# atx/padne

Measured on AMD Instinct MI355X. Metric: CG solves/s, higher is better.
Workload: dtype f64; 1 GPU; C4 8-layer N=10M: 8-layer jittered triangular Laplacian, 9999392 nodes, via-ring stitched, 1 A source/sink, amg-PCG to rtol 1e-12; n_unknowns=9999391, nnz_per_rank=69955225, rows_per_rank=9999391, parallelism=layer-partitioned x1

## Files before the change

padne_amd/csrc/pcg.hip:

```cpp
#include "common.hpp"

#include <algorithm>
#include <math.h>
#include <stdlib.h>
#include <string.h>
#include <vector>

namespace padne {

__device__ __forceinline__ double wave_sum_v(double v) {
#pragma unroll
    for (int off = 32; off > 0; off >>= 1) v += __shfl_down(v, off, 64);
    return v;
}

__device__ __forceinline__ double block_total(const double *__restrict__ partials, int P, double *red) {
    double s = 0.0;
    for (int i = threadIdx.x; i < P; i += 256) s += partials[i];
    s = wave_sum_v(s);
    const int lane = threadIdx.x & 63, w = threadIdx.x >> 6;
    if (lane == 0) red[w] = s;
    __syncthreads();
    const double t = (red[0] + red[1]) + (red[2] + red[3]);
    __syncthreads();
    return t;
}

__device__ __forceinline__ void block_total2(const double *__restrict__ pa, const int Pa, const double *__restrict__ pb, const int Pb,
                                             double *red2, double *ta, double *tb) {
    double sa = 0.0, sb = 0.0;
    const int P = Pa > Pb ? Pa : Pb;
    for (int i = threadIdx.x; i < P; i += 256) {
        if (i < Pa) sa += pa[i];
        if (i < Pb) sb += pb[i];
    }
    sa = wave_sum_v(sa);
    sb = wave_sum_v(sb);
    const int lane = threadIdx.x & 63, w = threadIdx.x >> 6;
    if (lane == 0) {
        red2[w] = sa;
        red2[4 + w] = sb;
    }
    __syncthreads();
    *ta = (red2[0] + red2[1]) + (red2[2] + red2[3]);
    *tb = (red2[4] + red2[5]) + (red2[6] + red2[7]);
    __syncthreads();
}

__device__ __forceinline__ void block_store_partial(double v, double *red, double *out) {
    v = wave_sum_v(v);
    const int lane = threadIdx.x & 63, w = threadIdx.x >> 6;
    if (lane == 0) red[w] = v;
    __syncthreads();
    if (threadIdx.x == 0) *out = (red[0] + red[1]) + (red[2] + red[3]);
    __syncthreads();
}

struct PcgStatus {
    int32_t done;
    int32_t code;
    int32_t iters;
    int32_t done_seen;
    double rr;
    double tol2;
    double bb;
};

__global__ __launch_bounds__(256) void pcg_init_kernel(
    const long long n, const double *__restrict__ b, const double *__restrict__ ax,
    const double *__restrict__ dinv, double *__restrict__ r, double *__restrict__ p,
    double *__restrict__ part_rz, double *__restrict__ part_rr, double *__restrict__ part_bb) {
    __shared__ double red[4];
    double rz = 0.0, rr = 0.0, bb = 0.0;
    for (long long i = (long long)blockIdx.x * 256 + threadIdx.x; i < n; i += (long long)gridDim.x * 256) {
        const double bi = b[i];
        const double ri = ax ? bi - ax[i] : bi;
        const double zi = dinv[i] * ri;
        r[i] = ri;
        p[i] = zi;
        rz += ri * zi;
        rr += ri * ri;
        bb += bi * bi;
    }
    block_store_partial(rz, red, part_rz + blockIdx.x);
    block_store_partial(rr, red, part_rr + blockIdx.x);
    block_store_partial(bb, red, part_bb + blockIdx.x);
}

__global__ __launch_bounds__(256) void fold_partials_kernel(const double *__restrict__ partials, int P,
                                                            int stride, int count, double *__restrict__ out) {
    __shared__ double red[4];
    for (int c = 0; c < count; ++c) {
        const double t = block_total(partials + (size_t)c * stride, P, red);
        if (threadIdx.x == 0) out[c] = t;
    }
}

__global__ void pcg_set_tolerance_kernel(PcgStatus *st, const double *__restrict__ scal_rr_bb, double rtol,
                                         double atol, int use_existing_bb) {
    const double bb = use_existing_bb ? st->bb : scal_rr_bb[1];
    const double rr = scal_rr_bb[0];
    double tol = rtol * sqrt(bb);
    if (atol > tol) tol = atol;
    st->bb = bb;
    st->tol2 = tol * tol;
    st->rr = rr;
    st->code = PADNE_OK;
    st->done = (rr <= tol * tol) ? 1 : 0;
    if (!(rr == rr)) {
        st->done = 1;
        st->code = PADNE_E_BREAKDOWN;
    }
}

__global__ __launch_bounds__(256) void pcg_update_xr_kernel(
    const long long n, const double *__restrict__ part_rz, const int P_rz,
    const double *__restrict__ part_pq, const int P_pq, const double *__restrict__ p,
    const double *__restrict__ q, const double *__restrict__ dinv, double *__restrict__ x,
    double *__restrict__ r, double *__restrict__ part_rz_new, double *__restrict__ part_rr,
    PcgStatus *__restrict__ st) {
    __shared__ double red[4];
    if (st->done) return;
    const double rz = block_total(part_rz, P_rz, red);
    const double pq = block_total(part_pq, P_pq, red);
    const double alpha = rz / pq;
    double s_rz = 0.0, s_rr = 0.0;
    for (long long i = (long long)blockIdx.x * 256 + threadIdx.x; i < n; i += (long long)gridDim.x * 256) {
        const double pi = p[i];
        const double ri = r[i] - alpha * q[i];
        if (x != nullptr) x[i] += alpha * pi;
        r[i] = ri;
        const double zi = dinv[i] * ri;
        s_rz += ri * zi;
        s_rr += ri * ri;
    }
    block_store_partial(s_rz, red, part_rz_new + blockIdx.x);
    block_store_partial(s_rr, red, part_rr + blockIdx.x);
}

__global__ __launch_bounds__(256) void pcg_update_p_kernel(
    const long long n, const double *__restrict__ part_rz_new, const double *__restrict__ part_rz_old,
    const int P_rz, const double *__restrict__ part_rr, const int P_rr,
    const double *__restrict__ part_pq, const int P_pq, const double *__restrict__ r,
    const double *__restrict__ dinv, double *__restrict__ p, PcgStatus *__restrict__ st,
    const int max_iter, double *__restrict__ rec_next = nullptr, double *__restrict__ rec_pq = nullptr) {
    __shared__ double red[4];
    if (st->done) return;
    const double rz_new = block_total(part_rz_new, P_rz, red);
    const double rz_old = block_total(part_rz_old, P_rz, red);
    const double beta = rz_new / rz_old;
    for (long long i = (long long)blockIdx.x * 256 + threadIdx.x; i < n; i += (long long)gridDim.x * 256) {
        p[i] = dinv[i] * r[i] + beta * p[i];
    }
    if (blockIdx.x == 0) {
        const double rr = block_total(part_rr, P_rr, red);
        const double pq = block_total(part_pq, P_pq, red);
        if (threadIdx.x == 0 && rec_next != nullptr) {
            rec_next[0] = rz_new;
            rec_next[1] = rr;
            rec_pq[0] = pq;
        }
        __syncthreads();
        if (threadIdx.x == 0) {
            const int it = st->iters + 1;
            st->iters = it;
            st->rr = rr;
            if (!(pq > 0.0) || !(rr == rr)) {
                st->code = PADNE_E_BREAKDOWN;
                st->done = 1;
            } else if (rr <= st->tol2 || it >= max_iter) {
                st->done = 1;
            }
        }
    }
}

__global__ __launch_bounds__(256) void residual_kernel(const long long n, const double *__restrict__ b,
                                                       const double *__restrict__ ax, double *__restrict__ r,
                                                       double *__restrict__ part_rr) {
    __shared__ double red[4];
    double rr = 0.0;
    for (long long i = (long long)blockIdx.x * 256 + threadIdx.x; i < n; i += (long long)gridDim.x * 256) {
        const double ri = ax[i] - b[i];
        if (r) r[i] = -ri;
        rr += ri * ri;
    }
    block_store_partial(rr, red, part_rr + blockIdx.x);
}

__global__ __launch_bounds__(256) void pcg_update_xr_plain_kernel(
    const long long n, const double *__restrict__ part_rz, const int P_rz, const double *__restrict__ part_pq,
    const int P_pq, const double *__restrict__ p, const double *__restrict__ q, double *__restrict__ x,
    double *__restrict__ r, double *__restrict__ part_rr, PcgStatus *__restrict__ st) {
    __shared__ double red[4];
    const int stop = st->done;
    if (blockIdx.x == 0 && threadIdx.x == 0) st->done_seen = stop;
    if (stop) return;
    const double rz = block_total(part_rz, P_rz, red);
    const double pq = block_total(part_pq, P_pq, red);
    const double alpha = rz / pq;
    double s_rr = 0.0;
    for (long long i = (long long)blockIdx.x * 256 + threadIdx.x; i < n; i += (long long)gridDim.x * 256) {
        const double ri = r[i] - alpha * q[i];
        x[i] += alpha * p[i];
        r[i] = ri;
        s_rr += ri * ri;
    }
    block_store_partial(s_rr, red, part_rr + blockIdx.x);
}

__global__ __launch_bounds__(256) void pcg_update_xr_entry_kernel(
    const long long n, const double *__restrict__ part_rz, const int P_rz, const double *__restrict__ part_pq,
    const int P_pq, const double *__restrict__ p, const double *__restrict__ q, double *__restrict__ x,
    double *__restrict__ r, double *__restrict__ part_rr, PcgStatus *__restrict__ st, const double *__restrict__ bb2,
    const float c, const float *__restrict__ dinv32, float *__restrict__ b32, float *__restrict__ xa32, const int p_hat) {
    __shared__ double red[8];
    const int stop = st->done;
    if (blockIdx.x == 0 && threadIdx.x == 0) st->done_seen = stop;
    if (stop) return;
    double rz, pq;
    block_total2(part_rz, P_rz, part_pq, P_pq, red, &rz, &pq);
    const double s2 = *bb2;
    const double s_inv = s2 > 0.0 ? 1.0 / sqrt(s2) : 1.0;
    const double alpha = p_hat ? rz / (pq * (s2 > 0.0 ? sqrt(s2) : 1.0)) : rz / pq;
    double s_rr = 0.0;
    for (long long i = (long long)blockIdx.x * 256 + threadIdx.x; i < n; i += (long long)gridDim.x * 256) {
        const double ri = r[i] - alpha * q[i];
        if (x != nullptr) x[i] += alpha * p[i];
        r[i] = ri;
        s_rr += ri * ri;
        const float v = (float)(ri * s_inv);
        b32[i] = v;
        if (xa32 != nullptr) xa32[i] = c * dinv32[i] * v;
    }
    block_store_partial(s_rr, red, part_rr + blockIdx.x);
}

__global__ void p_hat_from_z_kernel(const long long n, const double *__restrict__ z, const double *__restrict__ bb2, float *__restrict__ p32) {
    const double s2 = *bb2;
    const double s_inv = s2 > 0.0 ? 1.0 / sqrt(s2) : 1.0;
    for (long long i = (long long)blockIdx.x * blockDim.x + threadIdx.x; i < n; i += (long long)gridDim.x * blockDim.x)
        p32[i] = (float)(z[i] * s_inv);
}

__global__ __launch_bounds__(256) void pcg_update_p_z_kernel(
    const long long n, const double *__restrict__ part_rz_new, const double *__restrict__ part_rz_old,
    const int P_rz, const double *__restrict__ part_rr, const int P_rr, const double *__restrict__ part_pq,
    const int P_pq, const double *__restrict__ z, double *__restrict__ p, PcgStatus *__restrict__ st,
    const int max_iter, double *__restrict__ x_deferred, const float *__restrict__ z32, const double *__restrict__ bb2,
    float *__restrict__ p32, float *__restrict__ p32_next = nullptr, double *__restrict__ alpha_out = nullptr) {
    __shared__ double red[8];
    if (st->done_seen) return;
    double rz_new, rz_old;
    block_total2(part_rz_new, P_rz, part_rz_old, P_rz, red, &rz_new, &rz_old);
    const double beta = rz_new / rz_old;
    if (z32 != nullptr) {
        const double s2 = *bb2;
        const double z_mul = s2 > 0.0 ? sqrt(s2) : 1.0;
        const bool need_alpha = p32_next == nullptr || blockIdx.x == 0;
        const double alpha = need_alpha ? rz_old / block_total(part_pq, P_pq, red) : 0.0;
        if (p32 != nullptr) {
            const double alpha_hat = alpha / z_mul;
            if (p32_next != nullptr) {
                if (blockIdx.x == 0 && threadIdx.x == 0) *alpha_out = alpha_hat;
                for (long long i = (long long)blockIdx.x * 256 + threadIdx.x; i < n; i += (long long)gridDim.x * 256)
                    p32_next[i] = (float)((double)z32[i] + beta * (double)p32[i]);
            } else {
                for (long long i = (long long)blockIdx.x * 256 + threadIdx.x; i < n; i += (long long)gridDim.x * 256) {
                    const double pi = (double)p32[i];
                    x_deferred[i] += alpha_hat * pi;
                    p32[i] = (float)((double)z32[i] + beta * pi);
                }
            }
        } else {
            for (long long i = (long long)blockIdx.x * 256 + threadIdx.x; i < n; i += (long long)gridDim.x * 256) {
                const double pi = p[i];
                x_deferred[i] += alpha * pi;
                p[i] = (double)z32[i] * z_mul + beta * pi;
            }
        }
    } else if (x_deferred != nullptr) {
        const double alpha = rz_old / block_total(part_pq, P_pq, red);
        for (long long i = (long long)blockIdx.x * 256 + threadIdx.x; i < n; i += (long long)gridDim.x * 256) {
            const double pi = p[i];
            x_deferred[i] += alpha * pi;
            p[i] = z[i] + beta * pi;
        }
    } else {
        for (long long i = (long long)blockIdx.x * 256 + threadIdx.x; i < n; i += (long long)gridDim.x * 256)
            p[i] = z[i] + beta * p[i];
    }
    if (blockIdx.x == 0) {
        const double rr = block_total(part_rr, P_rr, red);
        const double pq = block_total(part_pq, P_pq, red);
        __syncthreads();
        if (threadIdx.x == 0) {
            const int it = st->iters + 1;
            st->iters = it;
            st->rr = rr;
            if (!(pq > 0.0) || !(rr == rr) || !(rz_new > 0.0)) {
                st->code = PADNE_E_BREAKDOWN;
                st->done = 1;
            } else if (rr <= st->tol2 || it >= max_iter) {
                st->done = 1;
            }
        }
    }
}

__global__ __launch_bounds__(256) void pcg_x_flush_kernel(const long long n, const float *__restrict__ hist, const size_t slot_stride,
                                                          const int n_slots, const double *__restrict__ alpha, const int j0,
                                                          const int j1, const PcgStatus *__restrict__ st, double *__restrict__ x) {
    __shared__ double a_s[64];
    __shared__ int s_s[64];
    const int hi = min(j1, st->iters);
    const int cnt = hi - j0;
    if (cnt <= 0) return;
    if ((int)threadIdx.x < cnt && threadIdx.x < 64) {
        a_s[threadIdx.x] = alpha[(j0 + threadIdx.x) % n_slots];
        s_s[threadIdx.x] = (j0 + threadIdx.x) % n_slots;
    }
    __syncthreads();
    for (long long i = (long long)blockIdx.x * 256 + threadIdx.x; i < n; i += (long long)gridDim.x * 256) {
        double xi = x[i];
        int k = 0;
        for (; k + 4 <= cnt; k += 4) {
            const float p0 = hist[(size_t)s_s[k] * slot_stride + i], p1 = hist[(size_t)s_s[k + 1] * slot_stride + i],
                        p2 = hist[(size_t)s_s[k + 2] * slot_stride + i], p3 = hist[(size_t)s_s[k + 3] * slot_stride + i];
            xi += a_s[k] * (double)p0;
            xi += a_s[k + 1] * (double)p1;
            xi += a_s[k + 2] * (double)p2;
            xi += a_s[k + 3] * (double)p3;
        }
        for (; k < cnt; ++k) xi += a_s[k] * (double)hist[(size_t)s_s[k] * slot_stride + i];
        x[i] = xi;
    }
}

__global__ __launch_bounds__(256) void pcg_init_plain_kernel(const long long n, const double *__restrict__ b,
                                                             const double *__restrict__ ax, double *__restrict__ r,
                                                             double *__restrict__ part_rr,
                                                             double *__restrict__ part_bb) {
    __shared__ double red[4];
    double rr = 0.0, bb = 0.0;
    for (long long i = (long long)blockIdx.x * 256 + threadIdx.x; i < n; i += (long long)gridDim.x * 256) {
        const double bi = b[i];
        const double ri = ax ? bi - ax[i] : bi;
        r[i] = ri;
        rr += ri * ri;
        bb += bi * bi;
    }
    block_store_partial(rr, red, part_rr + blockIdx.x);
    block_store_partial(bb, red, part_bb + blockIdx.x);
}

static int vec_grid(long long n) {
    long long g = (n + 255) / 256;
    if (g > 1024) g = 1024;
    if (g < 1) g = 1;
    return (int)g;
}

enum { SLOT_PQ = 0, SLOT_RZ0 = 1, SLOT_RZ1 = 2, SLOT_RR = 3, SLOT_BB = 4, SLOT_TMP = 5 };
static inline double *slot(padne_ctx *ctx, int s) { return ctx->partials + (size_t)s * kMaxPartials; }

template <typename T>
__global__ void halo_pack_kernel(T *__restrict__ v, const int *__restrict__ export_idx, int n_export,
                                 long long dst_offset, const int *__restrict__ done_flag) {
    if (done_flag != nullptr && *done_flag != 0) return;
    const int k = blockIdx.x * blockDim.x + threadIdx.x;
    if (k < n_export) v[dst_offset + k] = v[export_idx[k]];
}

enum { S_RR = 0, S_BB = 1, S_TRUE = 2,
       S_NRM = 3,
       S_PQ = 8, S_RZRR0 = 10, S_RZRR1 = 12 };

template <typename T>
__global__ void halo_store_peers_kernel(const T *__restrict__ v, const int *__restrict__ export_idx, int n_export, void *const *peers,
                                        size_t entry_off, int world, int rank, int m_cap, const int *__restrict__ done_flag,
                                        unsigned long long seq1) {
    if (done_flag != nullptr && *done_flag != 0) return;
    const int k = blockIdx.x * blockDim.x + threadIdx.x;
    if (k < n_export) {
        const T val = v[export_idx[k]];
        for (int q = 0; q < world; ++q) {
            T *cell = reinterpret_cast<T *>(static_cast<char *>(peers[q]) + entry_off + ((size_t)rank * m_cap + k) * 8);
            if (seq1 != 0ull)
                __hip_atomic_store(cell, val, __ATOMIC_RELAXED, __HIP_MEMORY_SCOPE_SYSTEM);
            else
                *cell = val;
        }
    }
    if (seq1 == 0ull) return;
    __threadfence_system();
    __syncthreads();
    __shared__ int s_last;
    if (threadIdx.x == 0) {
        unsigned int *counter = reinterpret_cast<unsigned int *>(static_cast<char *>(peers[rank]) + kP2pCounterOff);
        const unsigned int prev = __hip_atomic_fetch_add(counter, 1u, __ATOMIC_ACQ_REL, __HIP_MEMORY_SCOPE_AGENT);
        s_last = prev + 1u == gridDim.x ? 1 : 0;
        if (s_last) __hip_atomic_store(counter, 0u, __ATOMIC_RELAXED, __HIP_MEMORY_SCOPE_AGENT);
    }
    __syncthreads();
    if (s_last && (int)threadIdx.x < world) {
        unsigned long long *flag = reinterpret_cast<unsigned long long *>(static_cast<char *>(peers[threadIdx.x])) + rank;
        __hip_atomic_store(flag, seq1, __ATOMIC_RELEASE, __HIP_MEMORY_SCOPE_SYSTEM);
    }
}

template <typename T>
__global__ void halo_unpack_kernel(T *__restrict__ v, long long n_owned, int m, int world, const void *mbox, size_t entry_off,
                                   int m_cap, const int *__restrict__ done_flag, unsigned long long seq1,
                                   unsigned long long timeout_ticks) {
    if (done_flag != nullptr && *done_flag != 0) return;
    if (seq1 != 0ull) {
        if ((int)threadIdx.x < world) {
            const unsigned long long *flag = static_cast<const unsigned long long *>(mbox) + threadIdx.x;
            const unsigned long long t0 = wall_clock64();
            while (__hip_atomic_load(flag, __ATOMIC_ACQUIRE, __HIP_MEMORY_SCOPE_SYSTEM) < seq1) {
                if (wall_clock64() - t0 > timeout_ticks) {
                    unsigned long long *err = reinterpret_cast<unsigned long long *>(const_cast<char *>(static_cast<const char *>(mbox)) + kP2pErrorOff);
                    __hip_atomic_store(err, ((unsigned long long)(threadIdx.x + 1) << 48) | (seq1 & 0xffffffffffffull), __ATOMIC_RELAXED,
                                       __HIP_MEMORY_SCOPE_SYSTEM);
                    break;
                }
                __builtin_amdgcn_s_sleep(32);
            }
        }
        __syncthreads();
    }
    const int j = blockIdx.x * blockDim.x + threadIdx.x;
    if (j >= world * m) return;
    const int r = j / m, k = j - r * m;
    const T *cell = reinterpret_cast<const T *>(static_cast<const char *>(mbox) + entry_off + ((size_t)r * m_cap + k) * 8);
    v[n_owned + j] = seq1 != 0ull ? __hip_atomic_load(cell, __ATOMIC_RELAXED, __HIP_MEMORY_SCOPE_SYSTEM) : *cell;
}

template <typename T>
static int halo_send_t(padne_ctx *ctx, const HaloPlan &plan, T *v, const int32_t *done_flag, HaloTicket *tk) {
    tk->p2p = false;
    if (plan.m <= 0) return PADNE_OK;
    if (comm_p2p_enabled(ctx) && comm_p2p_fits(ctx, plan.m)) {
        void **peers = nullptr;
        PADNE_TRY(comm_p2p_begin(ctx, plan.m, &peers, &tk->entry_off));
        tk->p2p = true;
        tk->seq1 = ctx->p2p_ipc ? ctx->p2p_seq : 0ull;
        if (plan.n_export > 0 || ctx->p2p_ipc) {
            hipLaunchKernelGGL(halo_store_peers_kernel<T>, dim3(plan.n_export > 0 ? (plan.n_export + 255) / 256 : 1), dim3(256), 0,
                               ctx->stream, (const T *)v, plan.export_idx, plan.n_export, (void *const *)peers, tk->entry_off,
                               ctx->world, ctx->rank, ctx->p2p_m_cap, done_flag, tk->seq1);
            PADNE_HIP_CHECK(hipGetLastError());
        }
        return PADNE_OK;
    }
    const long long seg_off = plan.n_owned + (long long)ctx->rank * plan.m;
    if (plan.n_export > 0) {
        hipLaunchKernelGGL(halo_pack_kernel<T>, dim3((plan.n_export + 255) / 256), dim3(256), 0, ctx->stream, v,
                           plan.export_idx, plan.n_export, seg_off, done_flag);
        PADNE_HIP_CHECK(hipGetLastError());
    }
    return PADNE_OK;
}

static int allgather_t(padne_ctx *ctx, const double *send, double *recv, int count) { return comm_allgather_f64(ctx, send, recv, count); }
static int allgather_t(padne_ctx *ctx, const float *send, float *recv, int count) { return comm_allgather_f32(ctx, send, recv, count); }

template <typename T>
static int halo_recv_t(padne_ctx *ctx, const HaloPlan &plan, T *v, const int32_t *done_flag, const HaloTicket &tk) {
    if (plan.m <= 0) return PADNE_OK;
    if (tk.p2p) {
        PADNE_TRY(comm_p2p_arrive(ctx));
        const int n = ctx->world * plan.m;
        hipLaunchKernelGGL(halo_unpack_kernel<T>, dim3((n + 255) / 256), dim3(256), 0, ctx->stream, v, plan.n_owned, plan.m,
                           ctx->world, (const void *)ctx->p2p_mbox, tk.entry_off, ctx->p2p_m_cap, done_flag, tk.seq1,
                           (unsigned long long)ctx->p2p_timeout_ms * 100000ull);
        PADNE_HIP_CHECK(hipGetLastError());
        return PADNE_OK;
    }
    const long long seg_off = plan.n_owned + (long long)ctx->rank * plan.m;
    return allgather_t(ctx, v + seg_off, v + plan.n_owned, plan.m);
}

int halo_send(padne_ctx *ctx, const HaloPlan &plan, double *v, const int32_t *done_flag, HaloTicket *tk) { return halo_send_t(ctx, plan, v, done_flag, tk); }
int halo_send_f32(padne_ctx *ctx, const HaloPlan &plan, float *v, const int32_t *done_flag, HaloTicket *tk) { return halo_send_t(ctx, plan, v, done_flag, tk); }
int halo_recv(padne_ctx *ctx, const HaloPlan &plan, double *v, const int32_t *done_flag, const HaloTicket &tk) { return halo_recv_t(ctx, plan, v, done_flag, tk); }
int halo_recv_f32(padne_ctx *ctx, const HaloPlan &plan, float *v, const int32_t *done_flag, const HaloTicket &tk) { return halo_recv_t(ctx, plan, v, done_flag, tk); }

int halo_exchange_plan(padne_ctx *ctx, const HaloPlan &plan, double *v, const int32_t *done_flag) {
    HaloTicket tk;
    PADNE_TRY(halo_send(ctx, plan, v, done_flag, &tk));
    return halo_recv(ctx, plan, v, done_flag, tk);
}

int halo_exchange_plan_f32(padne_ctx *ctx, const HaloPlan &plan, float *v, const int32_t *done_flag) {
    HaloTicket tk;
    PADNE_TRY(halo_send_f32(ctx, plan, v, done_flag, &tk));
    return halo_recv_f32(ctx, plan, v, done_flag, tk);
}

static int halo_exchange(padne_ctx *ctx, double *v, const int32_t *done_flag) {
    if (!ctx->halo_on) return PADNE_OK;
    HaloPlan plan;
    plan.n_owned = ctx->halo_n_owned;
    plan.m = ctx->halo_m;
    plan.n_export = ctx->halo_n_export;
    plan.export_idx = ctx->halo_export;
    return halo_exchange_plan(ctx, plan, v, done_flag);
}

}
extern "C" int padne_ctx_halo_exchange_time(padne_ctx *ctx, int32_t repeats, double *seconds_out) {
    using namespace padne;
    PADNE_REQUIRE(ctx && seconds_out && repeats > 0, "argument");
    PADNE_REQUIRE(ctx->halo_on, "no halo plan on this context");
    PADNE_HIP_CHECK(hipSetDevice(ctx->device));
    const size_t n = (size_t)ctx->halo_n_owned + (size_t)ctx->world * (size_t)ctx->halo_m;
    double *v = (double *)pool_alloc(ctx, sizeof(double) * (n ? n : 1));
    if (v == nullptr) return PADNE_E_NOMEM;
    int rc = PADNE_OK;
    hipError_t e = hipMemsetAsync(v, 0, sizeof(double) * n, ctx->stream);
    for (int k = 0; k < 3 && rc == PADNE_OK && e == hipSuccess; ++k) rc = halo_exchange(ctx, v, nullptr);
    if (e == hipSuccess) e = hipEventRecord(ctx->ev0, ctx->stream);
    for (int k = 0; k < repeats && rc == PADNE_OK && e == hipSuccess; ++k) rc = halo_exchange(ctx, v, nullptr);
    if (e == hipSuccess) e = hipEventRecord(ctx->ev1, ctx->stream);
    if (e == hipSuccess) e = hipEventSynchronize(ctx->ev1);
    float ms = 0.f;
    if (e == hipSuccess) e = hipEventElapsedTime(&ms, ctx->ev0, ctx->ev1);
    pool_free(ctx, v);
    if (e != hipSuccess) {
        set_error("halo exchange timing failed: %s", hipGetErrorString(e));
        return PADNE_E_HIP;
    }
    PADNE_TRY(rc);
    PADNE_TRY(comm_p2p_check(ctx));
    *seconds_out = (double)ms * 1e-3 / repeats;
    return PADNE_OK;
}
extern "C" int padne_test_halo_exchange(padne_ctx *ctx, int32_t as_float, const double *x_host, double *out_host) {
    using namespace padne;
    PADNE_REQUIRE(ctx && x_host && out_host, "null argument");
    PADNE_REQUIRE(ctx->halo_on, "no halo plan on this context");
    PADNE_HIP_CHECK(hipSetDevice(ctx->device));
    const size_t n_owned = (size_t)ctx->halo_n_owned, n = n_owned + (size_t)ctx->world * (size_t)ctx->halo_m;
    const size_t elem = as_float ? sizeof(float) : sizeof(double);
    HaloPlan plan;
    plan.n_owned = ctx->halo_n_owned;
    plan.m = ctx->halo_m;
    plan.n_export = ctx->halo_n_export;
    plan.export_idx = ctx->halo_export;
    std::vector<float> h32(as_float ? n : 0);
    for (size_t i = 0; as_float && i < n_owned; ++i) h32[i] = (float)x_host[i];
    void *v = pool_alloc(ctx, elem * (n ? n : 1));
    if (v == nullptr) return PADNE_E_NOMEM;
    int rc = PADNE_OK;
    hipError_t e = hipMemsetAsync(v, 0xff, elem * n, ctx->stream);
    if (e == hipSuccess && n_owned > 0)
        e = hipMemcpyAsync(v, as_float ? (const void *)h32.data() : (const void *)x_host, elem * n_owned, hipMemcpyHostToDevice,
                           ctx->stream);
    if (e == hipSuccess) rc = as_float ? halo_exchange_plan_f32(ctx, plan, (float *)v, nullptr) : halo_exchange_plan(ctx, plan, (double *)v, nullptr);
    if (e == hipSuccess && rc == PADNE_OK && n > 0)
        e = hipMemcpyAsync(as_float ? (void *)h32.data() : (void *)out_host, v, elem * n, hipMemcpyDeviceToHost, ctx->stream);
    const hipError_t es = hipStreamSynchronize(ctx->stream);
    if (e == hipSuccess) e = es;
    pool_free(ctx, v);
    if (e != hipSuccess) {
        set_error("halo exchange failed: %s", hipGetErrorString(e));
        return PADNE_E_HIP;
    }
    PADNE_TRY(rc);
    PADNE_TRY(comm_p2p_check(ctx));
    for (size_t i = 0; as_float && i < n; ++i) out_host[i] = (double)h32[i];
    return PADNE_OK;
}
namespace padne {

static int halo_product_dot(padne_ctx *ctx, const padne_csr *a, double *v, double *q, double *partials, const int32_t *done_flag) {
    if (!ctx->halo_on) return launch_spmv(ctx, a, v, q, v, partials, done_flag);
    HaloPlan plan;
    plan.n_owned = ctx->halo_n_owned;
    plan.m = ctx->halo_m;
    plan.n_export = ctx->halo_n_export;
    plan.export_idx = ctx->halo_export;
    HaloTicket tk;
    PADNE_TRY(halo_send(ctx, plan, v, done_flag, &tk));
    const ProductArgs<double> dot{.dot_with = v, .partials = partials, .done_flag = done_flag};
    PADNE_TRY(launch_spmv<double, double>(ctx, a, SPMV_DOT, v, q, dot, SPMV_INTERIOR));
    PADNE_TRY(halo_recv(ctx, plan, v, done_flag, tk));
    return launch_spmv<double, double>(ctx, a, SPMV_DOT, v, q, dot, SPMV_BOUNDARY);
}

int amg_setup(padne_ctx *ctx, padne_csr *A0);
int amg_apply(padne_ctx *ctx, const padne_csr *A0, const double *r, double *z, double *partials_rz,
              const int32_t *done_flag, const double *bb2 = nullptr, bool entry_done = false, float *z32 = nullptr);
bool amg_f32_entry_args(const padne_csr *A0, float *jac, const float **dinv32, float **b32, float **xa32);
int amg_rz_partials(const padne_csr *A0);
void amg_info(const padne_csr *A0, int *levels, double *complexity, double *setup_seconds, long long *coarse_n);
const padne_csr *amg_level_matrix(const padne_csr *A0, int level, int which);

static thread_local bool t_last_solve_stagnated = false;
static thread_local bool t_last_solve_hit_cap = false;

struct EventList {
    std::vector<hipEvent_t> ev;
    ~EventList() { clear(); }
    void clear() {
        for (hipEvent_t e : ev) (void)hipEventDestroy(e);
        ev.clear();
    }
    bool empty() const { return ev.empty(); }
    size_t size() const { return ev.size(); }
    hipEvent_t operator[](size_t i) const { return ev[i]; }
    void push_back(hipEvent_t e) { ev.push_back(e); }
    hipEvent_t back() const { return ev.back(); }
};

static int solve_one(padne_ctx *ctx, const padne_csr *a, const padne_csr *prec, const double *b, double *x,
                     const padne_solve_opts *o, padne_solve_info *info, bool x_is_guess) {
    t_last_solve_stagnated = false;
    t_last_solve_hit_cap = false;
    const bool dist = comm_active(ctx);
    const bool halo = ctx->halo_on;
    const bool amg = prec != nullptr;
    const long long nr = a->n_rows;
    const long long n = halo ? ctx->halo_n_owned : nr;
    const long long nc = a->n_cols;
    if (halo) {
        PADNE_REQUIRE(nc == ctx->halo_n_owned + (long long)ctx->world * ctx->halo_m && nr <= nc,
                      "matrix shape does not match the halo plan");
    } else {
        PADNE_REQUIRE(nr == nc, "matrix must be square");
    }
    if (amg)
        PADNE_REQUIRE(prec->n_rows == n && (prec->n_cols == n || prec == a),
                      "preconditioner must be the matrix itself or its owned x owned block");
    constexpr int kXHist = 32;
    static_assert(kXHist <= 64, "pcg_x_flush_kernel holds the step lengths of one flush in 64 words of LDS");
    int n_hist = 0;
    if (amg && !dist && !halo && !ctx->opt.pcg_p64 && !ctx->opt.pcg_no_xhist && n > 0) {
        n_hist = (int)std::min<long long>(kXHist, std::max<long long>(8, ((long long)2 << 30) / (4 * n)));
        if (ctx->opt.force_xhist_small) n_hist = 8;
    }
    const size_t hist_stride = ((size_t)n + 63) & ~(size_t)63;
    const size_t base_bytes = (sizeof(double) * (size_t)(2 * n + 2 * nc + nr) + 4096 + 255) & ~(size_t)255;
    PADNE_TRY(ensure_workspace(ctx, base_bytes + (n_hist > 0 ? sizeof(float) * hist_stride * (size_t)n_hist + sizeof(double) * kXHist : 0)));
    double *r = (double *)ctx->ws;
    double *z = r + n;
    double *p = z + n;
    double *q = p + nc;
    double *xe = q + nr;
    PcgStatus *st = (PcgStatus *)ctx->status;
    PcgStatus *hst = (PcgStatus *)ctx->pinned;
    hipStream_t s = ctx->stream;
    const int gv = vec_grid(n);
    const int gs = spmv_partials(a);
    const int P_rz = amg ? amg_rz_partials(prec) : gv;
    const int max_iter = o->max_iter > 0 ? o->max_iter : 100000;
    const int check_every = o->check_every > 0 ? o->check_every : (amg ? 4 : 50);
    const int sample_stride = amg ? 4 : 16;
    double *scal = ctx->scalars;
    const double *bb_scalar = x_is_guess ? scal + S_NRM : scal + S_BB;
    float e_jac = 0.f;
    const float *e_dinv32 = nullptr;
    float *e_b32 = nullptr, *e_xa32 = nullptr;
    const bool fuse_entry = amg && amg_f32_entry_args(prec, &e_jac, &e_dinv32, &e_b32, &e_xa32);
    const bool defer_x = fuse_entry;
    float *z32 = defer_x && !dist && !halo ? (float *)z : nullptr;
    float *p32 = z32 != nullptr && spmv_x32_ok(a) ? (float *)p : nullptr;
    if (p32 == nullptr) n_hist = 0;
    float *hist = n_hist > 0 ? (float *)((char *)ctx->ws + base_bytes) : nullptr;
    double *alpha_hist = n_hist > 0 ? (double *)(hist + hist_stride * (size_t)n_hist) : nullptr;
    if (hist != nullptr) p32 = hist;
    auto p_place = [&](long long j) { return hist + hist_stride * (size_t)(j % n_hist); };

    PADNE_HIP_CHECK(hipMemsetAsync(st, 0, sizeof(PcgStatus), s));
    if (halo) PADNE_HIP_CHECK(hipMemsetAsync(p + n, 0, sizeof(double) * (size_t)(nc - n), s));
    PADNE_HIP_CHECK(hipEventRecord(ctx->ev0, s));

    auto product_Ax = [&](double *out) -> int {
        if (!halo) return launch_spmv(ctx, a, x, out, nullptr, nullptr, nullptr);
        PADNE_HIP_CHECK(hipMemcpyAsync(xe, x, sizeof(double) * (size_t)n, hipMemcpyDeviceToDevice, s));
        PADNE_HIP_CHECK(hipMemsetAsync(xe + n, 0, sizeof(double) * (size_t)(nc - n), s));
        PADNE_TRY(halo_exchange(ctx, xe, nullptr));
        return launch_spmv(ctx, a, xe, out, nullptr, nullptr, nullptr);
    };
    auto fold = [&](const double *first_slot, int P, long long stride, int count, double *out) -> int {
        hipLaunchKernelGGL(fold_partials_kernel, dim3(1), dim3(256), 0, s, first_slot, P, (int)stride, count, out);
        PADNE_HIP_CHECK(hipGetLastError());
        return PADNE_OK;
    };
    auto allreduce = [&](double *buf, int count) -> int { return dist ? comm_allreduce_sum_f64(ctx, buf, count) : PADNE_OK; };

    int restarts = 0, total_iters = 0, code = PADNE_OK;
    const bool sample_spmv = (o->flags & 2) != 0;
    EventList ev_a, ev_b;
    long long launched = 0;
    double true_rr = 0.0, bb = 0.0, tol2 = 0.0, prev_true_rr = 0.0;
    bool have_ax = false, stagnated = false;
    if (x_is_guess) {
        PADNE_TRY(product_Ax(q));
        have_ax = true;
    } else {
        PADNE_HIP_CHECK(hipMemsetAsync(x, 0, sizeof(double) * (size_t)n, s));
    }
    for (;;) {
        if (amg) {
            hipLaunchKernelGGL(pcg_init_plain_kernel, dim3(gv), dim3(256), 0, s, n, b, have_ax ? q : nullptr, r,
                               slot(ctx, SLOT_RR), slot(ctx, SLOT_BB));
            PADNE_HIP_CHECK(hipGetLastError());
            PADNE_TRY(fold(slot(ctx, SLOT_RR), gv, kMaxPartials, 2, scal + S_RR));
            PADNE_TRY(allreduce(scal + S_RR, 2));
            if (x_is_guess && restarts == 0)
                PADNE_HIP_CHECK(hipMemcpyAsync(scal + S_NRM, scal + S_RR, sizeof(double), hipMemcpyDeviceToDevice, s));
            PADNE_TRY(amg_apply(ctx, prec, r, z, slot(ctx, SLOT_RZ0), nullptr, bb_scalar));
            if (p32 != nullptr) {
                if (hist != nullptr) p32 = hist;
                hipLaunchKernelGGL(p_hat_from_z_kernel, dim3(gv), dim3(256), 0, s, n, (const double *)z, bb_scalar, p32);
                PADNE_HIP_CHECK(hipGetLastError());
            } else {
                PADNE_HIP_CHECK(hipMemcpyAsync(p, z, sizeof(double) * (size_t)n, hipMemcpyDeviceToDevice, s));
            }
        } else {
            hipLaunchKernelGGL(pcg_init_kernel, dim3(gv), dim3(256), 0, s, n, b, have_ax ? q : nullptr, a->dinv, r, p,
                               slot(ctx, SLOT_RZ0), slot(ctx, SLOT_RR), slot(ctx, SLOT_BB));
            PADNE_HIP_CHECK(hipGetLastError());
            PADNE_TRY(fold(slot(ctx, SLOT_RR), gv, kMaxPartials, 2, scal + S_RR));
            PADNE_TRY(allreduce(scal + S_RR, 2));
            if (x_is_guess && restarts == 0)
                PADNE_HIP_CHECK(hipMemcpyAsync(scal + S_NRM, scal + S_RR, sizeof(double), hipMemcpyDeviceToDevice, s));
        }
        if (dist) {
            PADNE_TRY(fold(slot(ctx, SLOT_RZ0), P_rz, kMaxPartials, 1, scal + S_RZRR0));
            PADNE_TRY(allreduce(scal + S_RZRR0, 1));
        }
        hipLaunchKernelGGL(pcg_set_tolerance_kernel, dim3(1), dim3(1), 0, s, st, scal + S_RR, o->rtol, o->atol,
                           restarts > 0 ? 1 : 0);
        PADNE_HIP_CHECK(hipGetLastError());
        int parity = 0;
        bool done = false;
        long long jq = 0, jf = 0;
        auto flush_x = [&]() -> int {
            if (hist == nullptr || jq == jf) return PADNE_OK;
            hipLaunchKernelGGL(pcg_x_flush_kernel, dim3(gv), dim3(256), 0, s, n, (const float *)hist, hist_stride, n_hist,
                               (const double *)alpha_hist, (int)jf, (int)jq, (const PcgStatus *)st, x);
            PADNE_HIP_CHECK(hipGetLastError());
            jf = jq;
            return PADNE_OK;
        };
        while (!done) {
            for (int k = 0; k < check_every; ++k) {
                const int rz_old_slot = parity ? SLOT_RZ1 : SLOT_RZ0;
                const int rz_new_slot = parity ? SLOT_RZ0 : SLOT_RZ1;
                double *s_old = scal + (parity ? S_RZRR1 : S_RZRR0);
                double *s_new = scal + (parity ? S_RZRR0 : S_RZRR1);
                const double *rz_old = dist ? s_old : slot(ctx, rz_old_slot);
                const double *rz_new = dist ? s_new : slot(ctx, rz_new_slot);
                const double *pq = dist ? scal + S_PQ : slot(ctx, SLOT_PQ);
                const double *rr = dist ? s_new + 1 : slot(ctx, SLOT_RR);
                const int Pz = dist ? 1 : P_rz, Pq = dist ? 1 : gs, Pr = dist ? 1 : gv;

                const bool sampled = sample_spmv && (launched++ % sample_stride) == 1 && ev_a.size() < 512;
                if (sampled) {
                    hipEvent_t e0, e1;
                    PADNE_HIP_CHECK(hipEventCreate(&e0));
                    PADNE_HIP_CHECK(hipEventCreate(&e1));
                    ev_a.push_back(e0);
                    ev_b.push_back(e1);
                    PADNE_HIP_CHECK(hipEventRecord(e0, s));
                }
                if (hist != nullptr) p32 = p_place(jq);
                if (p32 != nullptr)
                    PADNE_TRY(launch_spmv<double, double, float>(ctx, a, SPMV_DOT, p32, q,
                                                                 {.partials = slot(ctx, SLOT_PQ), .done_flag = &st->done}));
                else PADNE_TRY(halo_product_dot(ctx, a, p, q, slot(ctx, SLOT_PQ), &st->done));
                if (sampled) PADNE_HIP_CHECK(hipEventRecord(ev_b.back(), s));
                if (dist) {
                    PADNE_TRY(fold(slot(ctx, SLOT_PQ), gs, kMaxPartials, 1, scal + S_PQ));
                    PADNE_TRY(allreduce(scal + S_PQ, 1));
                }
                if (amg) {
                    if (fuse_entry)
                        hipLaunchKernelGGL(pcg_update_xr_entry_kernel, dim3(gv), dim3(256), 0, s, n, rz_old, Pz, pq, Pq, p, q,
                                           defer_x ? (double *)nullptr : x, r, slot(ctx, SLOT_RR), st, bb_scalar, e_jac, e_dinv32,
                                           e_b32, e_xa32, p32 != nullptr ? 1 : 0);
                    else
                        hipLaunchKernelGGL(pcg_update_xr_plain_kernel, dim3(gv), dim3(256), 0, s, n, rz_old, Pz, pq, Pq, p, q,
                                           x, r, slot(ctx, SLOT_RR), st);
                    PADNE_HIP_CHECK(hipGetLastError());
                    PADNE_TRY(amg_apply(ctx, prec, r, z, slot(ctx, rz_new_slot), &st->done, bb_scalar, fuse_entry, z32));
                    if (dist) {
                        PADNE_TRY(fold(slot(ctx, rz_new_slot), P_rz, kMaxPartials, 1, s_new));
                        PADNE_TRY(fold(slot(ctx, SLOT_RR), gv, kMaxPartials, 1, s_new + 1));
                        PADNE_TRY(allreduce(s_new, 2));
                    }
                    if (hist != nullptr) {
                        hipLaunchKernelGGL(pcg_update_p_z_kernel, dim3(gv), dim3(256), 0, s, n, rz_new, rz_old, Pz, rr, Pr,
                                           pq, Pq, z, p, st, max_iter - total_iters, (double *)nullptr, (const float *)z32,
                                           bb_scalar, p32, p_place(jq + 1), alpha_hist + (jq % n_hist));
                        ++jq;
                        if (jq - jf >= n_hist - 1) PADNE_TRY(flush_x());
                    } else {
                        hipLaunchKernelGGL(pcg_update_p_z_kernel, dim3(gv), dim3(256), 0, s, n, rz_new, rz_old, Pz, rr, Pr,
                                           pq, Pq, z, p, st, max_iter - total_iters, defer_x ? x : (double *)nullptr,
                                           (const float *)z32, bb_scalar, p32);
                    }
                } else {
                    hipLaunchKernelGGL(pcg_update_xr_kernel, dim3(gv), dim3(256), 0, s, n, rz_old, Pz, pq, Pq, p, q,
                                       a->dinv, x, r, slot(ctx, rz_new_slot), slot(ctx, SLOT_RR), st);
                    if (dist) {
                        PADNE_TRY(fold(slot(ctx, rz_new_slot), gv, (long long)(SLOT_RR - rz_new_slot) * kMaxPartials, 2,
                                       s_new));
                        PADNE_TRY(allreduce(s_new, 2));
                    }
                    hipLaunchKernelGGL(pcg_update_p_kernel, dim3(gv), dim3(256), 0, s, n, rz_new, rz_old, Pz, rr, Pr, pq,
                                       Pq, r, a->dinv, p, st, max_iter - total_iters);
                }
                parity ^= 1;
            }
            PADNE_HIP_CHECK(hipGetLastError());
            static_assert(sizeof(PcgStatus) <= 56, "one mailbox slot");
            PADNE_TRY(read_back(ctx, st, sizeof(PcgStatus), hst));
            done = hst->done != 0;
        }
        PADNE_TRY(flush_x());
        total_iters += hst->iters;
        code = hst->code;
        bb = hst->bb;
        tol2 = hst->tol2;
        PADNE_TRY(product_Ax(q));
        hipLaunchKernelGGL(residual_kernel, dim3(gv), dim3(256), 0, s, n, b, q, (double *)nullptr, slot(ctx, SLOT_TMP));
        PADNE_TRY(fold(slot(ctx, SLOT_TMP), gv, kMaxPartials, 1, scal + S_TRUE));
        PADNE_TRY(allreduce(scal + S_TRUE, 1));
        PADNE_TRY(read_back(ctx, scal + S_TRUE, sizeof(double), &true_rr));
        if (code != PADNE_OK) break;
        if (true_rr <= tol2 * 1.0000001 || total_iters >= max_iter || restarts >= 8) break;
        if (restarts > 0 && true_rr >= 0.25 * prev_true_rr) {
            stagnated = true;
            t_last_solve_stagnated = true;
            break;
        }
        prev_true_rr = true_rr;
        ++restarts;
        have_ax = true;
        PADNE_HIP_CHECK(hipMemsetAsync(st, 0, 4 * sizeof(int32_t), s));
    }
    t_last_solve_hit_cap = code == PADNE_OK && !stagnated && total_iters >= max_iter;
    PADNE_HIP_CHECK(hipEventRecord(ctx->ev1, s));
    PADNE_HIP_CHECK(hipEventSynchronize(ctx->ev1));
    PADNE_TRY(comm_p2p_check(ctx));
    float ms = 0.f;
    PADNE_HIP_CHECK(hipEventElapsedTime(&ms, ctx->ev0, ctx->ev1));
    if (!ev_a.empty()) {
        std::vector<double> t_s;
        for (size_t i = 0; i < ev_a.size(); ++i) {
            float t = 0.f;
            if (hipEventElapsedTime(&t, ev_a[i], ev_b[i]) == hipSuccess) t_s.push_back(t * 1e-3);
        }
        if (info && !t_s.empty()) {
            std::vector<double> sorted = t_s;
            std::sort(sorted.begin(), sorted.end());
            const double med = sorted[sorted.size() / 2];
            double sum = 0.0;
            int cnt = 0;
            for (double t : t_s)
                if (t >= 0.5 * med && t <= 2.0 * med) {
                    sum += t;
                    ++cnt;
                }
            if (cnt > 0) info->spmv_seconds = sum / cnt;
        }
    }
    if (info) {
        info->iterations += total_iters;
        info->restarts += restarts;
        const double rel = bb > 0 ? sqrt(true_rr / bb) : sqrt(true_rr);
        if (rel > info->rel_residual) info->rel_residual = rel;
        if (sqrt(true_rr) > info->abs_residual) info->abs_residual = sqrt(true_rr);
        info->solve_seconds += ms * 1e-3;
        if (code != PADNE_OK) info->status = code;
        else if (true_rr > tol2 * 1.0000001 && info->status == PADNE_OK) {
            if (!(stagnated && true_rr <= 100.0 * tol2)) info->status = PADNE_E_NOTCONVERGED;
        }
    }
    return PADNE_OK;
}

enum { SR_STATE = 0 , SR_RED = 4  };

__global__ __launch_bounds__(256) void sr_fold3_kernel(const double *__restrict__ p0, int n0, const double *__restrict__ p1,
                                                       int n1, const double *__restrict__ p2, int n2,
                                                       double *__restrict__ out) {
    __shared__ double red[4];
    const double *src = blockIdx.x == 0 ? p0 : (blockIdx.x == 1 ? p1 : p2);
    const int cnt = blockIdx.x == 0 ? n0 : (blockIdx.x == 1 ? n1 : n2);
    const double t = block_total(src, cnt, red);
    if (threadIdx.x == 0) out[blockIdx.x] = t;
}

__global__ __launch_bounds__(256) void sr_step_kernel(
    const long long n, double *__restrict__ sr, const double *__restrict__ z, const double *__restrict__ w,
    double *__restrict__ p, double *__restrict__ s, double *__restrict__ x, double *__restrict__ r,
    double *__restrict__ part_rr, PcgStatus *__restrict__ st, const int first, const int j, const int max_iter,
    const double *__restrict__ bb2, const float c, const float *__restrict__ dinv32, float *__restrict__ b32,
    float *__restrict__ xa32) {
    __shared__ double red[4];
    if (st->done) return;
    const double gn = sr[SR_RED + 0], delta = sr[SR_RED + 1], rr = sr[SR_RED + 2];
    const double *old = sr + SR_STATE + 2 * (j & 1);
    double alpha, beta = 0.0;
    if (first) {
        alpha = gn / delta;
    } else {
        beta = gn / old[0];
        alpha = gn / (delta - beta * gn / old[1]);
    }
    bool stop = !first && (rr <= st->tol2 || j >= max_iter);
    int code = PADNE_OK;
    if (!stop && (!(alpha > 0.0) || !(alpha == alpha) || !(gn > 0.0) || !(rr == rr))) {
        code = PADNE_E_BREAKDOWN;
        stop = true;
    }
    if (blockIdx.x == 0 && threadIdx.x == 0) {
        double *nw = sr + SR_STATE + 2 * ((j & 1) ^ 1);
        nw[0] = gn;
        nw[1] = alpha;
        if (!first) {
            st->iters = j;
            st->rr = rr;
        }
        if (code != PADNE_OK) st->code = code;
        if (stop) st->done = 1;
    }
    if (stop) return;
    double s_inv = 1.0;
    if (b32 != nullptr) {
        const double s2 = *bb2;
        s_inv = s2 > 0.0 ? 1.0 / sqrt(s2) : 1.0;
    }
    double s_rr = 0.0;
    for (long long i = (long long)blockIdx.x * 256 + threadIdx.x; i < n; i += (long long)gridDim.x * 256) {
        const double pi = first ? z[i] : z[i] + beta * p[i];
        const double si = first ? w[i] : w[i] + beta * s[i];
        p[i] = pi;
        s[i] = si;
        const double ri = r[i] - alpha * si;
        x[i] += alpha * pi;
        r[i] = ri;
        s_rr += ri * ri;
        if (b32 != nullptr) {
            const float v = (float)(ri * s_inv);
            b32[i] = v;
            if (xa32 != nullptr) xa32[i] = c * dinv32[i] * v;
        }
    }
    block_store_partial(s_rr, red, part_rr + blockIdx.x);
}


static int solve_one_single_reduction(padne_ctx *ctx, const padne_csr *a, const padne_csr *prec, const double *b,
                                      double *x, const padne_solve_opts *o, padne_solve_info *info, bool x_is_guess) {
    t_last_solve_stagnated = false;
    t_last_solve_hit_cap = false;
    const bool dist = comm_active(ctx);
    const bool halo = ctx->halo_on;
    const long long nr = a->n_rows;
    const long long n = halo ? ctx->halo_n_owned : nr;
    const long long nc = a->n_cols;
    if (halo) {
        PADNE_REQUIRE(nc == ctx->halo_n_owned + (long long)ctx->world * ctx->halo_m && nr <= nc,
                      "matrix shape does not match the halo plan");
    } else {
        PADNE_REQUIRE(nr == nc, "matrix must be square");
    }
    PADNE_REQUIRE(prec != nullptr && prec->n_rows == n && (prec->n_cols == n || prec == a),
                  "preconditioner must be the matrix itself or its owned x owned block");
    PADNE_TRY(ensure_workspace(ctx, sizeof(double) * (size_t)(3 * n + 2 * nc + 2 * nr) + 4096));
    double *r = (double *)ctx->ws;
    double *p = r + n;
    double *sv = p + n;
    double *z = sv + n;
    double *w = z + nc;
    double *q = w + nr;
    double *xe = q + nr;
    PcgStatus *st = (PcgStatus *)ctx->status;
    PcgStatus *hst = (PcgStatus *)ctx->pinned;
    hipStream_t s = ctx->stream;
    const int gv = vec_grid(n);
    const int gs = spmv_partials(a);
    const int P_rz = amg_rz_partials(prec);
    const int max_iter = o->max_iter > 0 ? o->max_iter : 100000;
    const int check_every = o->check_every > 0 ? o->check_every : 4;
    double *scal = ctx->scalars;
    double *sr = scal + 16;
    const double *bb_scalar = x_is_guess ? scal + S_NRM : scal + S_BB;
    float e_jac = 0.f;
    const float *e_dinv32 = nullptr;
    float *e_b32 = nullptr, *e_xa32 = nullptr;
    const bool fuse_entry = amg_f32_entry_args(prec, &e_jac, &e_dinv32, &e_b32, &e_xa32);

    PADNE_HIP_CHECK(hipMemsetAsync(st, 0, sizeof(PcgStatus), s));
    if (halo) PADNE_HIP_CHECK(hipMemsetAsync(z + n, 0, sizeof(double) * (size_t)(nc - n), s));
    PADNE_HIP_CHECK(hipEventRecord(ctx->ev0, s));
    auto product_Ax = [&](double *out) -> int {
        if (!halo) return launch_spmv(ctx, a, x, out, nullptr, nullptr, nullptr);
        PADNE_HIP_CHECK(hipMemcpyAsync(xe, x, sizeof(double) * (size_t)n, hipMemcpyDeviceToDevice, s));
        PADNE_HIP_CHECK(hipMemsetAsync(xe + n, 0, sizeof(double) * (size_t)(nc - n), s));
        PADNE_TRY(halo_exchange(ctx, xe, nullptr));
        return launch_spmv(ctx, a, xe, out, nullptr, nullptr, nullptr);
    };
    auto fold = [&](const double *first_slot, int P, long long stride, int count, double *out) -> int {
        hipLaunchKernelGGL(fold_partials_kernel, dim3(1), dim3(256), 0, s, first_slot, P, (int)stride, count, out);
        PADNE_HIP_CHECK(hipGetLastError());
        return PADNE_OK;
    };
    auto allreduce = [&](double *buf, int count) -> int { return dist ? comm_allreduce_sum_f64(ctx, buf, count) : PADNE_OK; };
    const bool sample_spmv = (o->flags & 2) != 0;
    EventList ev_a, ev_b;
    long long launched = 0;
    auto cycle_product_reduce = [&](bool entry_done, const int32_t *done_flag) -> int {
        PADNE_TRY(amg_apply(ctx, prec, r, z, slot(ctx, SLOT_RZ0), done_flag, bb_scalar, entry_done));
        const bool sampled = sample_spmv && (launched++ % 4) == 1 && ev_a.size() < 512;
        if (sampled) {
            hipEvent_t e0, e1;
            PADNE_HIP_CHECK(hipEventCreate(&e0));
            PADNE_HIP_CHECK(hipEventCreate(&e1));
            ev_a.push_back(e0);
            ev_b.push_back(e1);
            PADNE_HIP_CHECK(hipEventRecord(e0, s));
        }
        PADNE_TRY(halo_product_dot(ctx, a, z, w, slot(ctx, SLOT_PQ), done_flag));
        if (sampled) PADNE_HIP_CHECK(hipEventRecord(ev_b.back(), s));
        hipLaunchKernelGGL(sr_fold3_kernel, dim3(3), dim3(256), 0, s, slot(ctx, SLOT_RZ0), P_rz, slot(ctx, SLOT_PQ), gs,
                           slot(ctx, SLOT_RR), gv, sr + SR_RED);
        PADNE_HIP_CHECK(hipGetLastError());
        return allreduce(sr + SR_RED, 3);
    };

    int restarts = 0, total_iters = 0, code = PADNE_OK;
    double true_rr = 0.0, bb = 0.0, tol2 = 0.0, prev_true_rr = 0.0;
    bool have_ax = false, stagnated = false;
    if (x_is_guess) {
        PADNE_TRY(product_Ax(q));
        have_ax = true;
    } else {
        PADNE_HIP_CHECK(hipMemsetAsync(x, 0, sizeof(double) * (size_t)n, s));
    }
    for (;;) {
        hipLaunchKernelGGL(pcg_init_plain_kernel, dim3(gv), dim3(256), 0, s, n, b, have_ax ? q : nullptr, r,
                           slot(ctx, SLOT_RR), slot(ctx, SLOT_BB));
        PADNE_HIP_CHECK(hipGetLastError());
        PADNE_TRY(fold(slot(ctx, SLOT_RR), gv, kMaxPartials, 2, scal + S_RR));
        PADNE_TRY(allreduce(scal + S_RR, 2));
        if (x_is_guess && restarts == 0)
            PADNE_HIP_CHECK(hipMemcpyAsync(scal + S_NRM, scal + S_RR, sizeof(double), hipMemcpyDeviceToDevice, s));
        hipLaunchKernelGGL(pcg_set_tolerance_kernel, dim3(1), dim3(1), 0, s, st, scal + S_RR, o->rtol, o->atol,
                           restarts > 0 ? 1 : 0);
        PADNE_HIP_CHECK(hipGetLastError());
        PADNE_TRY(cycle_product_reduce(false, &st->done));
        int step_no = 0;
        hipLaunchKernelGGL(sr_step_kernel, dim3(gv), dim3(256), 0, s, n, sr, (const double *)z, (const double *)w, p, sv, x, r,
                           slot(ctx, SLOT_RR), st, 1, step_no, max_iter - total_iters, bb_scalar, e_jac, e_dinv32,
                           fuse_entry ? e_b32 : (float *)nullptr, e_xa32);
        PADNE_HIP_CHECK(hipGetLastError());
        bool done = false;
        while (!done) {
            for (int k = 0; k < check_every; ++k) {
                PADNE_TRY(cycle_product_reduce(fuse_entry, &st->done));
                ++step_no;
                hipLaunchKernelGGL(sr_step_kernel, dim3(gv), dim3(256), 0, s, n, sr, (const double *)z, (const double *)w, p, sv, x,
                                   r, slot(ctx, SLOT_RR), st, 0, step_no, max_iter - total_iters, bb_scalar, e_jac, e_dinv32,
                                   fuse_entry ? e_b32 : (float *)nullptr, e_xa32);
            }
            PADNE_HIP_CHECK(hipGetLastError());
            static_assert(sizeof(PcgStatus) <= 56, "one mailbox slot");
            PADNE_TRY(read_back(ctx, st, sizeof(PcgStatus), hst));
            done = hst->done != 0;
        }
        total_iters += hst->iters;
        code = hst->code;
        bb = hst->bb;
        tol2 = hst->tol2;
        PADNE_TRY(product_Ax(q));
        hipLaunchKernelGGL(residual_kernel, dim3(gv), dim3(256), 0, s, n, b, q, (double *)nullptr, slot(ctx, SLOT_TMP));
        PADNE_TRY(fold(slot(ctx, SLOT_TMP), gv, kMaxPartials, 1, scal + S_TRUE));
        PADNE_TRY(allreduce(scal + S_TRUE, 1));
        PADNE_TRY(read_back(ctx, scal + S_TRUE, sizeof(double), &true_rr));
        if (code != PADNE_OK) break;
        if (true_rr <= tol2 * 1.0000001 || total_iters >= max_iter || restarts >= 8) break;
        if (restarts > 0 && true_rr >= 0.25 * prev_true_rr) {
            stagnated = true;
            t_last_solve_stagnated = true;
            break;
        }
        prev_true_rr = true_rr;
        ++restarts;
        have_ax = true;
        PADNE_HIP_CHECK(hipMemsetAsync(st, 0, 4 * sizeof(int32_t), s));
    }
    t_last_solve_hit_cap = code == PADNE_OK && !stagnated && total_iters >= max_iter;
    PADNE_HIP_CHECK(hipEventRecord(ctx->ev1, s));
    PADNE_HIP_CHECK(hipEventSynchronize(ctx->ev1));
    PADNE_TRY(comm_p2p_check(ctx));
    float ms = 0.f;
    PADNE_HIP_CHECK(hipEventElapsedTime(&ms, ctx->ev0, ctx->ev1));
    if (!ev_a.empty()) {
        std::vector<double> t_s;
        for (size_t i = 0; i < ev_a.size(); ++i) {
// ... 934 lines not shown
```

Before: 32.07 solves/s.

## Decide PCG convergence before AMG apply and prefetch vectors ahead of reductions

Adds a single-block decide kernel that runs right after the x/r update. It reduces rr, pq and rz, writes alpha, and sets done before the AMG preconditioner is applied, so a converged final iteration can skip the V-cycle work gated on the done flag. The update kernels now load their first-row operands before the partial-sum reduction to hide load latency, and reductions prefetch all partials into registers. The p-update kernel gains a 'last' path that only flushes x. This adds one small kernel launch per iteration and makes the status-flag handshake more complex.

After: 32.82 solves/s (median of 6 runs). +2.3%, better.

```diff
diff --git a/padne_amd/csrc/pcg.hip b/padne_amd/csrc/pcg.hip
--- a/padne_amd/csrc/pcg.hip
+++ b/padne_amd/csrc/pcg.hip
@@ -26,24 +26,32 @@
     return t;
 }
 
-__device__ __forceinline__ void block_total2(const double *__restrict__ pa, const int Pa, const double *__restrict__ pb, const int Pb,
-                                             double *red2, double *ta, double *tb) {
-    double sa = 0.0, sb = 0.0;
-    const int P = Pa > Pb ? Pa : Pb;
-    for (int i = threadIdx.x; i < P; i += 256) {
-        if (i < Pa) sa += pa[i];
-        if (i < Pb) sb += pb[i];
-    }
-    sa = wave_sum_v(sa);
-    sb = wave_sum_v(sb);
+template <int K>
+__device__ __forceinline__ void block_totals_ahead(const double *const (&pa)[K], const int (&P)[K], double *red, double (&t)[K]) {
+    constexpr int J = kMaxPartials / 256;
+    double v[K][J];
+#pragma unroll
+    for (int k = 0; k < K; ++k) {
+#pragma unroll
+        for (int j = 0; j < J; ++j) {
+            const int i = threadIdx.x + 256 * j;
+            v[k][j] = pa[k][i < P[k] ? i : 0];
+        }
+    }
     const int lane = threadIdx.x & 63, w = threadIdx.x >> 6;
-    if (lane == 0) {
-        red2[w] = sa;
-        red2[4 + w] = sb;
+#pragma unroll
+    for (int k = 0; k < K; ++k) {
+        double s = 0.0;
+#pragma unroll
+        for (int j = 0; j < J; ++j)
+            if ((int)threadIdx.x + 256 * j < P[k]) s += v[k][j];
+        for (int i = threadIdx.x + 256 * J; i < P[k]; i += 256) s += pa[k][i];
+        s = wave_sum_v(s);
+        if (lane == 0) red[4 * k + w] = s;
     }
     __syncthreads();
-    *ta = (red2[0] + red2[1]) + (red2[2] + red2[3]);
-    *tb = (red2[4] + red2[5]) + (red2[6] + red2[7]);
+#pragma unroll
+    for (int k = 0; k < K; ++k) t[k] = (red[4 * k] + red[4 * k + 1]) + (red[4 * k + 2] + red[4 * k + 3]);
     __syncthreads();
 }
 
@@ -218,22 +226,66 @@
     const int stop = st->done;
     if (blockIdx.x == 0 && threadIdx.x == 0) st->done_seen = stop;
     if (stop) return;
-    double rz, pq;
-    block_total2(part_rz, P_rz, part_pq, P_pq, red, &rz, &pq);
+    const long long i0 = (long long)blockIdx.x * 256 + threadIdx.x;
+    double r0 = 0.0, q0 = 0.0;
+    if (i0 < n) {
+        r0 = r[i0];
+        q0 = q[i0];
+    }
+    const double *const parts[2] = {part_rz, part_pq};
+    const int counts[2] = {P_rz, P_pq};
+    double tot[2];
+    block_totals_ahead<2>(parts, counts, red, tot);
+    const double rz = tot[0], pq = tot[1];
     const double s2 = *bb2;
     const double s_inv = s2 > 0.0 ? 1.0 / sqrt(s2) : 1.0;
     const double alpha = p_hat ? rz / (pq * (s2 > 0.0 ? sqrt(s2) : 1.0)) : rz / pq;
     double s_rr = 0.0;
-    for (long long i = (long long)blockIdx.x * 256 + threadIdx.x; i < n; i += (long long)gridDim.x * 256) {
-        const double ri = r[i] - alpha * q[i];
+    auto row = [&](const long long i, const double r_old, const double qi) {
+        const double ri = r_old - alpha * qi;
         if (x != nullptr) x[i] += alpha * p[i];
         r[i] = ri;
         s_rr += ri * ri;
         const float v = (float)(ri * s_inv);
         b32[i] = v;
         if (xa32 != nullptr) xa32[i] = c * dinv32[i] * v;
-    }
+    };
+    if (i0 < n) row(i0, r0, q0);
+    for (long long i = i0 + (long long)gridDim.x * 256; i < n; i += (long long)gridDim.x * 256) row(i, r[i], q[i]);
     block_store_partial(s_rr, red, part_rr + blockIdx.x);
+}
+
+__global__ __launch_bounds__(256) void pcg_decide_kernel(
+    const double *__restrict__ part_rz, const int P_rz, const double *__restrict__ part_pq, const int P_pq,
+    const double *__restrict__ part_rr, const int P_rr, PcgStatus *__restrict__ st, const int max_iter,
+    const double *__restrict__ bb2, double *__restrict__ alpha_out) {
+    __shared__ double red[12];
+    if (st->done) return;
+    const double *const parts[3] = {part_rr, part_pq, part_rz};
+    const int counts[3] = {P_rr, P_pq, P_rz};
+    double tot[3];
+    block_totals_ahead<3>(parts, counts, red, tot);
+    const double rr = tot[0], pq = tot[1];
+    if (alpha_out != nullptr) {
+        const double rz = tot[2];
+        const double s2 = *bb2;
+        const double z_mul = s2 > 0.0 ? sqrt(s2) : 1.0;
+        const double alpha = rz / pq;
+        if (threadIdx.x == 0) *alpha_out = alpha / z_mul;
+    }
+    if (threadIdx.x == 0) {
+        const int it = st->iters + 1;
+        st->iters = it;
+        st->rr = rr;
+        if (!(pq > 0.0) || !(rr == rr)) {
+            st->code = PADNE_E_BREAKDOWN;
+            st->done = 1;
+            st->done_seen = 2;
+        } else if (rr <= st->tol2 || it >= max_iter) {
+            st->done = 1;
+            st->done_seen = 2;
+        }
+    }
 }
 
 __global__ void p_hat_from_z_kernel(const long long n, const double *__restrict__ z, const double *__restrict__ bb2, float *__restrict__ p32) {
@@ -248,22 +300,49 @@
     const int P_rz, const double *__restrict__ part_rr, const int P_rr, const double *__restrict__ part_pq,
     const int P_pq, const double *__restrict__ z, double *__restrict__ p, PcgStatus *__restrict__ st,
     const int max_iter, double *__restrict__ x_deferred, const float *__restrict__ z32, const double *__restrict__ bb2,
-    float *__restrict__ p32, float *__restrict__ p32_next = nullptr, double *__restrict__ alpha_out = nullptr) {
+    float *__restrict__ p32, float *__restrict__ p32_next = nullptr, double *__restrict__ alpha_out = nullptr,
+    const int decided = 0) {
     __shared__ double red[8];
-    if (st->done_seen) return;
-    double rz_new, rz_old;
-    block_total2(part_rz_new, P_rz, part_rz_old, P_rz, red, &rz_new, &rz_old);
+    const int seen = st->done_seen;
+    if (seen == 1) return;
+    const bool last = seen == 2;
+    if (last && x_deferred == nullptr) return;
+    const long long i0 = (long long)blockIdx.x * 256 + threadIdx.x;
+    const bool ahead = p32_next != nullptr && i0 < n;
+    float z0 = 0.f, p0 = 0.f;
+    if (ahead) {
+        z0 = z32[i0];
+        p0 = p32[i0];
+    }
+    const double *const parts[2] = {part_rz_new, part_rz_old};
+    const int counts[2] = {P_rz, P_rz};
+    double tot[2];
+    block_totals_ahead<2>(parts, counts, red, tot);
+    asm volatile("" : "+v"(z0), "+v"(p0));
+    const double rz_new = tot[0], rz_old = tot[1];
     const double beta = rz_new / rz_old;
+    if (last) {
+        const double s2 = *bb2;
+        const double z_mul = s2 > 0.0 ? sqrt(s2) : 1.0;
+        const double alpha = rz_old / block_total(part_pq, P_pq, red);
+        const double alpha_hat = alpha / z_mul;
+        for (long long i = i0; i < n; i += (long long)gridDim.x * 256) {
+            if (p32 != nullptr) x_deferred[i] += alpha_hat * (double)p32[i];
+            else x_deferred[i] += alpha * p[i];
+        }
+        return;
+    }
     if (z32 != nullptr) {
         const double s2 = *bb2;
         const double z_mul = s2 > 0.0 ? sqrt(s2) : 1.0;
-        const bool need_alpha = p32_next == nullptr || blockIdx.x == 0;
+        const bool need_alpha = p32_next == nullptr || (blockIdx.x == 0 && !decided);
         const double alpha = need_alpha ? rz_old / block_total(part_pq, P_pq, red) : 0.0;
         if (p32 != nullptr) {
             const double alpha_hat = alpha / z_mul;
             if (p32_next != nullptr) {
-                if (blockIdx.x == 0 && threadIdx.x == 0) *alpha_out = alpha_hat;
-                for (long long i = (long long)blockIdx.x * 256 + threadIdx.x; i < n; i += (long long)gridDim.x * 256)
+                if (blockIdx.x == 0 && threadIdx.x == 0 && !decided) *alpha_out = alpha_hat;
+                if (ahead) p32_next[i0] = (float)((double)z0 + beta * (double)p0);
+                for (long long i = i0 + (long long)gridDim.x * 256; i < n; i += (long long)gridDim.x * 256)
                     p32_next[i] = (float)((double)z32[i] + beta * (double)p32[i]);
             } else {
                 for (long long i = (long long)blockIdx.x * 256 + threadIdx.x; i < n; i += (long long)gridDim.x * 256) {
@@ -290,7 +369,12 @@
         for (long long i = (long long)blockIdx.x * 256 + threadIdx.x; i < n; i += (long long)gridDim.x * 256)
             p[i] = z[i] + beta * p[i];
     }
-    if (blockIdx.x == 0) {
+    if (decided) {
+        if (blockIdx.x == 0 && threadIdx.x == 0 && !(rz_new > 0.0)) {
+            st->code = PADNE_E_BREAKDOWN;
+            st->done = 1;
+        }
+    } else if (blockIdx.x == 0) {
         const double rr = block_total(part_rr, P_rr, red);
         const double pq = block_total(part_pq, P_pq, red);
         __syncthreads();
@@ -671,6 +755,7 @@
     float *hist = n_hist > 0 ? (float *)((char *)ctx->ws + base_bytes) : nullptr;
     double *alpha_hist = n_hist > 0 ? (double *)(hist + hist_stride * (size_t)n_hist) : nullptr;
     if (hist != nullptr) p32 = hist;
+    const bool decide_early = z32 != nullptr;
     auto p_place = [&](long long j) { return hist + hist_stride * (size_t)(j % n_hist); };
 
     PADNE_HIP_CHECK(hipMemsetAsync(st, 0, sizeof(PcgStatus), s));
@@ -787,6 +872,12 @@
                         hipLaunchKernelGGL(pcg_update_xr_plain_kernel, dim3(gv), dim3(256), 0, s, n, rz_old, Pz, pq, Pq, p, q,
                                            x, r, slot(ctx, SLOT_RR), st);
                     PADNE_HIP_CHECK(hipGetLastError());
+                    if (decide_early) {
+                        hipLaunchKernelGGL(pcg_decide_kernel, dim3(1), dim3(256), 0, s, rz_old, Pz, pq, Pq, rr, Pr, st,
+                                           max_iter - total_iters, bb_scalar,
+                                           hist != nullptr ? alpha_hist + (jq % n_hist) : (double *)nullptr);
+                        PADNE_HIP_CHECK(hipGetLastError());
+                    }
                     PADNE_TRY(amg_apply(ctx, prec, r, z, slot(ctx, rz_new_slot), &st->done, bb_scalar, fuse_entry, z32));
                     if (dist) {
                         PADNE_TRY(fold(slot(ctx, rz_new_slot), P_rz, kMaxPartials, 1, s_new));
@@ -796,13 +887,14 @@
                     if (hist != nullptr) {
                         hipLaunchKernelGGL(pcg_update_p_z_kernel, dim3(gv), dim3(256), 0, s, n, rz_new, rz_old, Pz, rr, Pr,
                                            pq, Pq, z, p, st, max_iter - total_iters, (double *)nullptr, (const float *)z32,
-                                           bb_scalar, p32, p_place(jq + 1), alpha_hist + (jq % n_hist));
+                                           bb_scalar, p32, p_place(jq + 1), alpha_hist + (jq % n_hist), decide_early ? 1 : 0);
                         ++jq;
                         if (jq - jf >= n_hist - 1) PADNE_TRY(flush_x());
                     } else {
                         hipLaunchKernelGGL(pcg_update_p_z_kernel, dim3(gv), dim3(256), 0, s, n, rz_new, rz_old, Pz, rr, Pr,
                                            pq, Pq, z, p, st, max_iter - total_iters, defer_x ? x : (double *)nullptr,
-                                           (const float *)z32, bb_scalar, p32);
+                                           (const float *)z32, bb_scalar, p32, (float *)nullptr, (double *)nullptr,
+                                           decide_early ? 1 : 0);
                     }
                 } else {
                     hipLaunchKernelGGL(pcg_update_xr_kernel, dim3(gv), dim3(256), 0, s, n, rz_old, Pz, pq, Pq, p, q,
```
